# ksil/LFPSQP.jl

Measured on AMD Instinct MI355X. Metric: projected-CG iters/sec at n=1e7, m=128 fp64, higher is better.
Workload: dtype f64

## Files before the change

lfpsqp.jl_amd/csrc/context.hip:

```cpp
#include <dlfcn.h>
#include <stdarg.h>
#include <stdio.h>
#include <stdlib.h>
#include <ctype.h>
#include <string.h>

#include <algorithm>

#include "internal.h"

namespace lfpsqp {

int set_err(lfpsqp_ctx* ctx, int code, const char* fmt, ...) {
    char buf[1024];
    va_list ap;
    va_start(ap, fmt);
    vsnprintf(buf, sizeof(buf), fmt, ap);
    va_end(ap);
    if (ctx) ctx->err = buf;
    else fprintf(stderr, "lfpsqp: %s\n", buf);
    return code;
}

static int regrow(lfpsqp_ctx* ctx, double** buf, size_t* have, size_t cap, bool zero) {
// ... 222 lines not shown
}

__global__ __launch_bounds__(lfpsqp::kThreads) void view_copy_kernel(const double* __restrict__ A, const double* __restrict__ rs, const double* __restrict__ u,
                                                                     const double* __restrict__ w, double* __restrict__ D, int64_t ld, int64_t n, int m) {
    const int64_t i = ((int64_t)blockIdx.x * lfpsqp::kThreads + threadIdx.x) * 2;
    if (i >= n) return;
    const double2 s = rs ? lfpsqp::ld2(rs + i) : make_double2(1.0, 1.0);
    const double2 uu = u ? lfpsqp::ld2(u + i) : make_double2(0.0, 0.0);
    const bool v1 = i + 1 < n;
    const int j0 = blockIdx.y * 16, j1 = (j0 + 16 < m) ? j0 + 16 : m;
#pragma unroll 4
    for (int j = j0; j < j1; ++j) {
        const double2 c = lfpsqp::ld2(A + (int64_t)j * ld + i);
        const double wj = u ? w[j] : 0.0;
        const double2 o = make_double2(fma(uu.x, wj, s.x * c.x), fma(uu.y, wj, s.y * c.y));
        if (v1) lfpsqp::st2(D + (int64_t)j * ld + i, o);
        else D[(int64_t)j * ld + i] = o.x;
    }
}

extern "C" {

int lfpsqp_ctx_create(int device, lfpsqp_ctx** out) {
    if (!out) return LFPSQP_ERR_ARG;
    *out = nullptr;
    int ndev = 0;
    if (hipGetDeviceCount(&ndev) != hipSuccess || ndev <= 0) return set_err(nullptr, LFPSQP_ERR_HIP, "no HIP device visible");
    if (device < 0 || device >= ndev) return set_err(nullptr, LFPSQP_ERR_ARG, "device %d out of range (%d visible)", device, ndev);
    lfpsqp_ctx* ctx = new lfpsqp_ctx();
    ctx->device = device;
    if (hipSetDevice(device) != hipSuccess) { delete ctx; return set_err(nullptr, LFPSQP_ERR_HIP, "hipSetDevice(%d) failed", device); }
    hipDeviceProp_t prop;
    if (hipGetDeviceProperties(&prop, device) == hipSuccess) {
        ctx->devname = std::string(prop.name) + " (" + prop.gcnArchName + ")";
        ctx->num_cu = prop.multiProcessorCount;
        ctx->real_gpu = strncmp(prop.gcnArchName, "gfx", 3) == 0;
    }
    bool ok = hipStreamCreate(&ctx->stream) == hipSuccess;
    ok = ok && hipMalloc((void**)&ctx->scal, 64 * sizeof(double)) == hipSuccess;
    ok = ok && hipMalloc((void**)&ctx->istat, 128 * sizeof(int64_t)) == hipSuccess;
    ok = ok && hipHostMalloc((void**)&ctx->h_scal, 4 * 64 * sizeof(double)) == hipSuccess;
    ok = ok && hipHostMalloc((void**)&ctx->h_istat, 4 * 16 * sizeof(int64_t)) == hipSuccess;
    for (int i = 0; ok && i < 4; ++i) ok = hipEventCreate(&ctx->ev_slot[i]) == hipSuccess;
    ok = ok && hipEventCreate(&ctx->ev_t0) == hipSuccess && hipEventCreate(&ctx->ev_t1) == hipSuccess;
    if (ok) ok = hipMemset(ctx->scal, 0, 64 * sizeof(double)) == hipSuccess && hipMemset(ctx->istat, 0, 128 * sizeof(int64_t)) == hipSuccess;
    if (!ok) { delete ctx; return set_err(nullptr, LFPSQP_ERR_HIP, "context resource allocation failed"); }
    if (const char* e = getenv("LFPSQP_ONEPASS")) ctx->tune_onepass = atoi(e);
    if (const char* e = getenv("LFPSQP_SPGRAM")) ctx->tune_spgram = atoi(e) < 0 ? -1 : 0;
    if (const char* e = getenv("LFPSQP_VEC_BLOCKS")) ctx->tune_vec_blocks = atoi(e) > 0 ? atoi(e) : 0;
    if (const char* e = getenv("LFPSQP_NRB_MFMA")) ctx->tune_nrb_mfma = atoi(e) > 0 ? 1 : (atoi(e) < 0 ? -1 : 0);
    if (const char* e = getenv("LFPSQP_GPING")) ctx->tune_gping = atoi(e) == 1 ? 1 : 0;
    if (const char* e = getenv("LFPSQP_NRB_WG_CAP")) ctx->batch_wg_cap = atoi(e) > 0 ? atoi(e) : 0;
    if (const char* e = getenv("LFPSQP_STAGE_ROUNDS")) ctx->stage_cap = atoi(e) > 0 ? atoi(e) : 0;
    *out = ctx;
    return 0;
}

int lfpsqp_ctx_destroy(lfpsqp_ctx* ctx) {
    if (!ctx) return 0;
    (void)hipSetDevice(ctx->device);
    (void)hipStreamSynchronize(ctx->stream);
    if (ctx->comm.kind == Comm::RCCL && ctx->comm.nccl_comm && ctx->comm.ncclCommDestroy) ctx->comm.ncclCommDestroy(ctx->comm.nccl_comm);
    for (int r = 0; r < kP2PMaxRanks; ++r)
        if (ctx->comm.p2p_peer[r] && ctx->comm.p2p_peer[r] != ctx->comm.p2p_mine) (void)hipIpcCloseMemHandle(ctx->comm.p2p_peer[r]);
    if (ctx->comm.p2p_mine) (void)hipFree(ctx->comm.p2p_mine);
    if (ctx->comm.p2p_err) (void)hipHostFree(ctx->comm.p2p_err);
    if (ctx->prof_init)
        for (int s = 0; s < kProfSlots; ++s)
            for (int e = 0; e < kProfEvents; ++e)
                for (int k = 0; k < 2; ++k) (void)hipEventDestroy(ctx->prof_ev[s][e][k]);
    for (int i = 0; i < 4; ++i) if (ctx->ev_slot[i]) (void)hipEventDestroy(ctx->ev_slot[i]);
    if (ctx->ev_t0) (void)hipEventDestroy(ctx->ev_t0);
    if (ctx->ev_t1) (void)hipEventDestroy(ctx->ev_t1);
    if (ctx->part) (void)hipFree(ctx->part);
    if (ctx->small) (void)hipFree(ctx->small);
    if (ctx->d_m) (void)hipFree(ctx->d_m);
    if (ctx->d_qw) (void)hipFree(ctx->d_qw);
    if (ctx->d_zeros) (void)hipFree(ctx->d_zeros);
    if (ctx->d_nvec) (void)hipFree(ctx->d_nvec);
    if (ctx->d_tri) (void)hipFree(ctx->d_tri);
    if (ctx->d_view) (void)hipFree(ctx->d_view);
    if (ctx->h_m) (void)hipHostFree(ctx->h_m);
    if (ctx->scal) (void)hipFree(ctx->scal);
    if (ctx->istat) (void)hipFree(ctx->istat);
    if (ctx->h_scal) (void)hipHostFree(ctx->h_scal);
    if (ctx->h_istat) (void)hipHostFree(ctx->h_istat);
    if (ctx->stream) (void)hipStreamDestroy(ctx->stream);
    delete ctx;
    return 0;
}

int lfpsqp_ctx_sync(lfpsqp_ctx* ctx) {
    LF_ARG(ctx, ctx != nullptr);
    LF_HIP(ctx, hipStreamSynchronize(ctx->stream));
    return 0;
}

const char* lfpsqp_last_error(const lfpsqp_ctx* ctx) { return ctx ? ctx->err.c_str() : "null context"; }

int lfpsqp_device_name(const lfpsqp_ctx* ctx, char* buf, int64_t buflen) {
    if (!ctx || !buf || buflen <= 0) return LFPSQP_ERR_ARG;
    snprintf(buf, (size_t)buflen, "%s", ctx->devname.c_str());
    return 0;
}

int lfpsqp_device_uuid(const lfpsqp_ctx* ctx, char* buf, int64_t buflen) {
// ... 588 lines not shown
```

lfpsqp.jl_amd/csrc/internal.h:

```cpp
#pragma once
#include <hip/hip_runtime.h>
#include <stdint.h>

#include <string>
#include <vector>

#include "../../include/lfpsqp_hip.h"
#include "kernels.h"

struct lfpsqp_slab {
    void* p = nullptr;
    int refs = 0;
};
struct lfpsqp_vec {
    double* p = nullptr;
    int64_t n = 0;
    int64_t cap = 0;
    lfpsqp_slab* slab = nullptr;
};

constexpr int64_t kLdSkewDefault = 16;

struct lfpsqp_mat {
    double* p = nullptr;
    int64_t n = 0, m = 0;
    int64_t ld = 0;
    const double* rs = nullptr;
    const double* ru = nullptr;
    const double* rw = nullptr;
    bool view = false;
    lfpsqp_mat plain() const { lfpsqp_mat q = *this; q.rs = q.ru = q.rw = nullptr; q.view = false; return q; }
};

namespace lfpsqp {

constexpr int kProfSlots = 8;
constexpr int kProfEvents = 128;

struct Comm {
    int rank = 0, nranks = 1;
    enum Kind { NONE, RCCL, CALLBACK, P2P } kind = NONE;
    void* p2p_mine = nullptr;
    void* p2p_peer[16] = {nullptr};
    uint64_t p2p_seq = 0;
    int* p2p_err = nullptr;
    int p2p_memkind = 0;
    bool p2p_allow_coarse = false;
    void* rccl_lib = nullptr;
    void* nccl_comm = nullptr;
    int (*ncclAllReduce)(const void*, void*, size_t, int , int , void*, hipStream_t) = nullptr;
    int (*ncclCommDestroy)(void*) = nullptr;
    const char* (*ncclGetErrorString)(int) = nullptr;
    lfpsqp_allreduce_fn cb = nullptr;
    void* cb_user = nullptr;
};

}

struct lfpsqp_ctx {
    int device = 0;
    int num_cu = 0;
    hipStream_t stream = nullptr;
    std::string err;
    std::string devname;
    lfpsqp::Comm comm;
    bool comm_active() const { return comm.kind != lfpsqp::Comm::NONE; }

    double* part = nullptr;
    size_t part_cap = 0;
    double* small = nullptr;
    size_t small_cap = 0;
    double* d_m = nullptr;
    double* h_m = nullptr;
    size_t m_cap = 0;
    std::vector<double> warm_V;
    int warm_m = 0;
    double* d_view = nullptr;
    double* d_nvec = nullptr;
    size_t nvec_cap = 0;
    double* d_tri = nullptr;
    size_t tri_cap = 0;
    double* d_zeros = nullptr;
    double* d_qw = nullptr;
    size_t qw_cap = 0;
    double* scal = nullptr;
    int64_t* istat = nullptr;
    double* h_scal = nullptr;
    int64_t* h_istat = nullptr;
    hipEvent_t ev_slot[4] = {nullptr, nullptr, nullptr, nullptr};
    hipEvent_t ev_t0 = nullptr, ev_t1 = nullptr;

    int tune_ks = 0;
    bool tune_nt = true;
    int ks_for(int64_t n) const { return tune_ks ? tune_ks : (n >= 4000000 ? 4 : 2); }
    int tune_onepass = 0;
    int tune_spgram = 0;
    int tune_vec_blocks = 0;
    int tune_nrb_mfma = -1;
    int tune_gping = 0;

    bool real_gpu = false;
    int place_tries = 3;
    int64_t place_min_bytes = (int64_t)1 << 30;
    double place_last_ms[64] = {0};
    int place_last_n = 0, place_last_pick = 0;

    struct ProjcgResume {
        bool valid = false;
        const double *x = nullptr, *g = nullptr, *d = nullptr, *Z = nullptr;
        int m = 0;
        int64_t nv = 0, iters = 0;
        bool gcur_is_rp = false;
        const double *dg = nullptr, *b = nullptr;
        double a0 = 0.0;
        int64_t n_global = 0;
        uint64_t epoch = 0;
    } pcg_resume;
    int batch_wg_cap = 0;
    int stage_cap = 0;
    uint64_t launch_epoch = 0;

    bool profiling = false;
    hipEvent_t prof_ev[lfpsqp::kProfSlots][lfpsqp::kProfEvents][2];
    int prof_used[lfpsqp::kProfSlots] = {0};
    int64_t prof_seq[lfpsqp::kProfSlots] = {0};
    bool prof_live[lfpsqp::kProfSlots] = {false};
    int64_t prof_count[lfpsqp::kProfSlots] = {0};
    double prof_ms[lfpsqp::kProfSlots] = {0};
    bool prof_init = false;
};

namespace lfpsqp {

int set_err(lfpsqp_ctx* ctx, int code, const char* fmt, ...);
int ensure_part(lfpsqp_ctx* ctx, size_t doubles);
int ensure_small(lfpsqp_ctx* ctx, size_t doubles);
int ensure_tri(lfpsqp_ctx* ctx, size_t doubles);
int ensure_mvec(lfpsqp_ctx* ctx, size_t doubles);
int ensure_nvec(lfpsqp_ctx* ctx, size_t doubles);

struct Layout {
    struct Region { double** p; size_t at; };
    Region r[12];
    int k = 0;
    size_t n = 0;
    size_t skip(size_t len, size_t align = 2) {
        const size_t at = (n + align - 1) / align * align;
        n = at + len;
        return at;
    }
    void add(double*& p, size_t len, size_t align = 2) { r[k++] = Region{&p, skip(len, align)}; }
    size_t size() const { return n; }
    void carve(double* base) const { for (int i = 0; i < k; ++i) *r[i].p = base + r[i].at; }
};
int ensure_view(lfpsqp_ctx* ctx);
constexpr int kViewTau = 8;
constexpr int kViewScratch = kViewTau + 4 * 1024 + 64;
int allreduce_dev(lfpsqp_ctx* ctx, double* buf, int64_t count, int op = 0);

void prof_begin(lfpsqp_ctx* ctx, int s);
void prof_end(lfpsqp_ctx* ctx, int s);
void prof_collect(lfpsqp_ctx* ctx);

inline int64_t round_up(int64_t a, int64_t b) { return (a + b - 1) / b * b; }
inline int64_t ntiles_of(int64_t n, int ks) { return (n + (int64_t)kSlabRows * ks - 1) / ((int64_t)kSlabRows * ks); }

#define LF_HIP(ctx, expr)                                                                              \
    do {                                                                                               \
        hipError_t e__ = (expr);                                                                       \
        if (e__ != hipSuccess)                                                                         \
            return lfpsqp::set_err((ctx), LFPSQP_ERR_HIP, "%s failed: %s (%s:%d)", #expr,              \
                                   hipGetErrorString(e__), __FILE__, __LINE__);                        \
// ... 376 lines not shown
```

lfpsqp.jl_amd/csrc/projcg.hip:

```cpp
#include <math.h>
#include <stdlib.h>

#include <algorithm>
#include <vector>

#include "internal.h"
#include "sparse.h"
#include "sphess.h"

namespace lfpsqp {

enum { S_DAD = 0, S_RG = 1, S_ALPHA = 2, S_RPGP = 3, S_GPGP = 4, S_BETA = 5, S_NR = 6, S_TOL = 7, S_DD = 8, S_ALPHA_PREV = 9 };
enum { I_STATUS = 0, I_ITER = 1, I_MAXIT = 2 };
enum { ST_RUNNING = 0, ST_CONVERGED = 1, ST_RG_BREAK = 2, ST_NEGCURV = 3, ST_MAXIT = 4 };

struct AOpD {
    double a0;
    const double* dg;
    __device__ __forceinline__ double2 apply(int64_t i, double2 d) const {
        if (dg) {
            const double2 q = ld2(dg + i);
            return make_double2((a0 + q.x) * d.x, (a0 + q.y) * d.y);
        }
        return make_double2(a0 * d.x, a0 * d.y);
    }
};

struct AOpV {
    const double* Av;
    __device__ __forceinline__ double2 apply(int64_t i, double2) const { return ld2(Av + i); }
};

struct AOpLR {
    double a0;
    const double* dg;
    const double* V;
    int64_t ldv;
    int k;
    const double *sigma, *vtv;
    __device__ __forceinline__ double2 apply(int64_t i, double2 d) const {
        double2 o = dg ? make_double2((a0 + dg[i]) * d.x, (a0 + dg[i + 1]) * d.y) : make_double2(a0 * d.x, a0 * d.y);
        for (int j = 0; j < k; ++j) {
            const double c = ld_scal(sigma + j) * ld_scal(vtv + j);
            const double2 v = ld2(V + (int64_t)j * ldv + i);
            o.x = fma(v.x, c, o.x);
            o.y = fma(v.y, c, o.y);
        }
        return o;
    }
};

template <int B>
struct BandD {
    static_assert(B >= 1 && B <= 4, "bandwidth 1 .. 4");
    double a0;
    const double* dg;
// ... 352 lines not shown
    int first;
    __device__ __forceinline__ bool skip() const { return ld_stat(istat + I_STATUS) != ST_RUNNING; }
    __device__ __forceinline__ void apply(int64_t i, bool v0, bool v1, double* red) const {
        double2 dd = ld2(d + i);
        if (!first) {
            const double alpha = ld_scal(scal + S_ALPHA);
            double2 xx = ld2(x + i);
            xx = make_double2(fma(alpha, dd.x, xx.x), fma(alpha, dd.y, xx.y));
            if (v1) st2(x + i, xx);
            else if (v0) x[i] = xx.x;
            const double beta = ld_scal(scal + S_BETA);
            const double2 gg = ld2(g + i);
            dd = make_double2(beta * dd.x - gg.x, beta * dd.y - gg.y);
            if (v1) st2(d + i, dd);
            else if (v0) d[i] = dd.x;
        }
        const double2 ad = A.apply(i, dd);
        double s = 0.0;
        if (v0) s = dd.x * ad.x;
        if (v1) s = fma(dd.y, ad.y, s);
        red[0] += s;
    }
};
struct PcgDirX {
    double* d;
    const double* g;
    double* x;
    const double* scal;
    const int64_t* istat;
    __device__ __forceinline__ bool skip() const { return ld_stat(istat + I_STATUS) != ST_RUNNING; }
    __device__ __forceinline__ void apply(int64_t i, bool v0, bool v1, double*) const {
        const double alpha = ld_scal(scal + S_ALPHA), beta = ld_scal(scal + S_BETA);
        double2 dd = ld2(d + i), xx = ld2(x + i);
        const double2 gg = ld2(g + i);
        xx = make_double2(fma(alpha, dd.x, xx.x), fma(alpha, dd.y, xx.y));
        dd = make_double2(beta * dd.x - gg.x, beta * dd.y - gg.y);
        if (v1) { st2(x + i, xx); st2(d + i, dd); }
        else if (v0) { x[i] = xx.x; d[i] = dd.x; }
    }
};
struct DotPairF {
    const double* a;
    const double* b;
    const int64_t* istat;
    __device__ __forceinline__ bool skip() const { return ld_stat(istat + I_STATUS) != ST_RUNNING; }
    __device__ __forceinline__ void apply(int64_t i, bool v0, bool v1, double* red) const {
        const double2 x = ld2(a + i), y = ld2(b + i);
        double s = 0.0;
        if (v0) s = x.x * y.x;
        if (v1) s = fma(x.y, y.y, s);
        red[0] += s;
    }
};
constexpr int kRing = 8, kRingOff = 8;
struct HostMirror {
    int64_t* hstat;
    double* hnr;
    __device__ __forceinline__ void publish(int64_t status, int64_t iter, double nr) const {
        __hip_atomic_store(hnr, nr, __ATOMIC_RELAXED, __HIP_MEMORY_SCOPE_SYSTEM);
        __hip_atomic_store(hstat + 1, iter, __ATOMIC_RELAXED, __HIP_MEMORY_SCOPE_SYSTEM);
        __hip_atomic_store(hstat + kRingOff + (iter % kRing), status, __ATOMIC_RELAXED, __HIP_MEMORY_SCOPE_SYSTEM);
        __hip_atomic_store(hstat, status, __ATOMIC_RELEASE, __HIP_MEMORY_SCOPE_SYSTEM);
    }
};

struct PcgPost1 {
    double* scal;
    int64_t* istat;
    HostMirror hm;
    __device__ __forceinline__ bool skip() const { return ld_stat(istat + I_STATUS) != ST_RUNNING; }
    __device__ __forceinline__ void run(double*) const {
        const int64_t it = ld_stat(istat + I_ITER) + 1;
        istat[I_ITER] = it;
        const double dAd = ld_scal(scal + S_DAD), rg = ld_scal(scal + S_RG);
        if (dAd <= 0.0) { istat[I_STATUS] = ST_NEGCURV; hm.publish(ST_NEGCURV, it, ld_scal(scal + S_NR)); }
        else if (rg <= 0.0) { istat[I_STATUS] = ST_RG_BREAK; hm.publish(ST_RG_BREAK, it, ld_scal(scal + S_NR)); }
        else scal[S_ALPHA] = rg / dAd;
    }
};

template <class AOP>
struct PcgStepV {
    const double* d;
    const double* g;
    AOP A;
    const double* scal;
    const int64_t* istat;
    __device__ __forceinline__ bool skip() const { return ld_stat(istat + I_STATUS) != ST_RUNNING; }
    __device__ __forceinline__ double2 rp_at(int64_t r) const {
        const double alpha = ld_scal(scal + S_ALPHA);
        const double2 dd = ld2(d + r), gg = ld2(g + r);
        const double2 ad = A.apply(r, dd);
        return make_double2(fma(alpha, ad.x, gg.x), fma(alpha, ad.y, gg.y));
    }
    __device__ __forceinline__ double2 load(int64_t r, bool v0, bool v1) const {
        const double2 rr = rp_at(r);
        return make_double2(v0 ? rr.x : 0.0, v1 ? rr.y : 0.0);
    }
};

template <class AOP>
struct PcgProjE {
    const double* rp;
    double* g;
    double* d;
    const int64_t* istat;
    int init;
    PcgStepV<AOP> sv;
    __device__ __forceinline__ bool skip() const { return ld_stat(istat + I_STATUS) != ST_RUNNING; }
    __device__ __forceinline__ void apply(int64_t r, double2 acc, bool v0, bool v1, double* red) const {
        const double2 rr = init ? ld2(rp + r) : sv.rp_at(r);
        const double2 gp = make_double2(rr.x - acc.x, rr.y - acc.y);
        if (v1) st2(g + r, gp);
        else if (v0) g[r] = gp.x;
        if (init) {
// ... 434 lines not shown
            else if (gpgp <= 0.0) st = ST_RG_BREAK;
            else {
                u.scal[S_ALPHA_PREV] = (u.init == 2) ? 0.0 : ld_scal(u.scal + S_ALPHA);
                u.scal[S_ALPHA] = gpgp / dAd_next;
            }
            if (st != ST_RUNNING) u.hm.publish(st, it + 1, nr);
        }
        if (st != ST_RUNNING) u.istat[I_STATUS] = st;
        go = (st == ST_RUNNING);
        sh[0] = gpgp / dAd_next;
        sh[1] = beta;
        if (go)
            for (int j = 0; j < u.k; ++j) {
                const double vg = ld_scal(S + 5 + j);
                const double vd = (u.init == 1) ? -vg : fma(beta, u.vdraw[j], -vg);
                u.vdraw[j] = vd;
                u.vdc[j] = ld_scal(u.sigma + j) * vd;
            }
    }
    __syncthreads();
    if (!go) return;
    const double alpha = sh[0], beta = sh[1];
    for (int j = threadIdx.x; j < u.m; j += blockDim.x) {
        const double t1 = ld_scal(u.T + j);
        double t2 = ld_scal(u.T + u.m + j);
        if (u.triM) t2 -= s_mu[j];
        for (int l = 0; l < u.k; ++l)
            t2 = fma(u.UtV[(size_t)l * u.m + j], ld_scal(u.sigma + l) * ld_scal(u.T + 2 * u.m + 5 + l), t2);
        const double t3 = (u.init == 1) ? -t2 : fma(beta, u.t3[j], -t2);
        u.t3[j] = t3;
        const double ut = fma(alpha, t3, t1);
        u.Utr[j] = ut;
        if (u.W) s_utr[j] = ut;
    }
    if (u.W) {
        __syncthreads();
        const double* const xin[1] = {nullptr};
        double yo[1];
        small_wdot<1>(u.W, 1, (size_t)u.wm, u.wm, u.m, xin, s_utr, yo, s_part);
        int rp = 32;
        while (rp < u.wm) rp <<= 1;
        if ((int)threadIdx.x < u.wm && (int)threadIdx.x / rp == 0) u.uA[threadIdx.x] = yo[0];
    }
}
#ifndef LFPSQP_K1_NT
#define LFPSQP_K1_NT 1
#endif
struct PcgDirG {
    double* d;
    const double* g;
    double* x;
    const double* scal;
    const int64_t* istat;
    int force;
    __device__ __forceinline__ bool skip() const { return !force && ld_stat(istat + I_STATUS) != ST_RUNNING; }
    __device__ __forceinline__ void apply(int64_t i, bool v0, bool v1, double*) const {
        double2 dd = ld2(d + i);
        if (!force) {
            const double alpha = ld_scal(scal + S_ALPHA_PREV);
            double2 xx = ld2(x + i);
            xx = make_double2(fma(alpha, dd.x, xx.x), fma(alpha, dd.y, xx.y));
            if (v1) { if (LFPSQP_K1_NT >= 1) st2_stream(x + i, xx); else st2(x + i, xx); }
            else if (v0) x[i] = xx.x;
        }
        const double beta = ld_scal(scal + S_BETA);
        const double2 gg = ld2(g + i);
        dd = make_double2(beta * dd.x - gg.x, beta * dd.y - gg.y);
        if (v1) { if (LFPSQP_K1_NT == 1) st2_stream(d + i, dd); else st2(d + i, dd); }
        else if (v0) d[i] = dd.x;
    }
};

template <class AOP>
struct ResidualV {
    const double* x;
    const double* b;
    double* out;
    AOP A;
    double sgn;
    __device__ __forceinline__ bool skip() const { return false; }
    __device__ __forceinline__ double2 load(int64_t r, bool v0, bool v1) const {
        const double2 xx = ld2(x + r), bb = ld2(b + r);
        const double2 ax = A.apply(r, xx);
        const double2 rr = make_double2(sgn * (ax.x - bb.x), sgn * (ax.y - bb.y));
        if (out) {
            if (v1) st2(out + r, rr);
            else if (v0) out[r] = rr.x;
        }
        return make_double2(v0 ? rr.x : 0.0, v1 ? rr.y : 0.0);
    }
};
struct InitState {
    double* scal;
    int64_t* istat;
    double tol;
    int64_t maxit;
    __device__ __forceinline__ bool skip() const { return false; }
    __device__ __forceinline__ void run(double*) const {
        for (int k = 0; k < 16; ++k) scal[k] = 0.0;
        scal[S_TOL] = tol;
        scal[S_NR] = INFINITY;
        istat[I_STATUS] = ST_RUNNING;
        istat[I_ITER] = 0;
        istat[I_MAXIT] = maxit;
    }
};
struct FlushXF {
    double* x;
    const double* d;
    const double* scal;
    __device__ __forceinline__ bool skip() const { return false; }
    __device__ __forceinline__ void apply(int64_t i, bool v0, bool v1, double*) const {
        const double alpha = ld_scal(scal + S_ALPHA);
        const double2 dd = ld2(d + i);
        double2 xx = ld2(x + i);
        xx = make_double2(fma(alpha, dd.x, xx.x), fma(alpha, dd.y, xx.y));
        if (v1) st2(x + i, xx);
        else if (v0) x[i] = xx.x;
    }
};
// ... 341 lines not shown
    static CoupledOp sparse_of(const char* who, double a0, const lfpsqp_vec* dg, const lfpsqp_sphess* S) {
        return CoupledOp{SPARSE, who, a0, dg, nullptr, 0, S->n, S->Kr, {}, S};
    }
    static CoupledOp banded(const char* who, double a0, const lfpsqp_vec* dg, const double* off, int64_t ld, int64_t rows, int bw) {
        return CoupledOp{BAND, who, a0, dg, off, ld, rows, bw, {1, 2, 3, 4}};
    }
};
template <typename F>
static int with_diags(const CoupledOp& A, F&& fn) {
    return A.wide() ? fn(std::integral_constant<int, kDiagsWide>{}) : fn(std::integral_constant<int, kDiagsNarrow>{});
}
template <typename F>
static int with_gathers(const CoupledOp& A, int64_t n, int64_t nc, F&& fn) {
    if (A.kind == CoupledOp::SPARSE) return fn(A.sparse(n, nc));
    return with_diags(A, [&](auto Cc) -> int { return fn(A.template diags<decltype(Cc)::value>(n, nc)); });
}
template <typename F>
static int with_band(int bw, F&& fn) {
    switch (bw) {
        case 1: return fn(std::integral_constant<int, 1>{});
        case 2: return fn(std::integral_constant<int, 2>{});
        case 3: return fn(std::integral_constant<int, 3>{});
        default: return fn(std::integral_constant<int, 4>{});
    }
}

static int coupled_mul(lfpsqp_ctx* ctx, const CoupledOp& A, int64_t n, int64_t nc, const double* v, double* out) {
    if (A.kind != CoupledOp::BAND)
        return with_gathers(A, n, nc, [&](auto Ad) -> int {
            using D = decltype(Ad);
            return run_vec<DiagsMulF<D>, 0, NoPost>(ctx, n, DiagsMulF<D>{Ad, v, out, nullptr}, 0u, nullptr, NoPost());
        });
    return with_band(A.K, [&](auto Bc) -> int {
        constexpr int B = decltype(Bc)::value;
        return run_vec<TriMulF<B>, 0, NoPost>(ctx, n, TriMulF<B>{A.template band<B>(n, nc), v, out, nullptr}, 0u, nullptr, NoPost());
    });
}
template <typename F>
static int with_stacked_init(bool stacked, bool init, F&& fn) {
    if (stacked) return init ? fn(std::true_type{}, std::true_type{}) : fn(std::true_type{}, std::false_type{});
    return init ? fn(std::false_type{}, std::true_type{}) : fn(std::false_type{}, std::false_type{});
}

struct PcgOperator {
    enum Kind { DIAGONAL, CALLBACK, LOWRANK, COUPLED } kind;
    lfpsqp_diag_op diag;
    lfpsqp_opfun fn = nullptr;
    void* user = nullptr;
    const lfpsqp_lowrank_op* lr = nullptr;
    const CoupledOp* cp = nullptr;
    lfpsqp_vec* Av = nullptr;
};

static int projcg_impl(lfpsqp_ctx* ctx, lfpsqp_vec* x, lfpsqp_vec* lambda, const PcgOperator& op, const lfpsqp_basis* U, const lfpsqp_vec* b,
                       const lfpsqp_vec* c, double tol, int64_t maxit, int64_t n_global, int flags, const lfpsqp_projcg_work* work,
                       int64_t* iters, double* nr) {
    const bool callback = op.kind == PcgOperator::CALLBACK;
    const lfpsqp_lowrank_op* LRop = op.kind == PcgOperator::LOWRANK ? op.lr : nullptr;
    const CoupledOp* cop = op.kind == PcgOperator::COUPLED ? op.cp : nullptr;
    const lfpsqp_diag_op* A = &op.diag;
    lfpsqp_vec* Av = op.Av;
    LF_ARG(ctx, ctx && x && U && b && work && iters && nr);
    if (callback || cop) {
        LF_ARG(ctx, Av && Av->n == b->n && !(flags & (LFPSQP_PROJCG_RESUME | (cop ? 0 : LFPSQP_PROJCG_START_GIVEN) | LFPSQP_PROJCG_START_PROJECTED)));
    }
    LF_ARG(ctx, !((flags & LFPSQP_PROJCG_RESUME) && (flags & (LFPSQP_PROJCG_START_GIVEN | LFPSQP_PROJCG_START_PROJECTED))));
    LF_ARG(ctx, !((flags & LFPSQP_PROJCG_START_GIVEN) && (flags & LFPSQP_PROJCG_START_PROJECTED)));
    LF_ARG(ctx, work->g && work->d && work->rp && work->Utr);
    const lfpsqp_ctx::ProjcgResume rs = ctx->pcg_resume;
    const bool stacked = U->Dx != nullptr;
    const int64_t nv = b->n;
    const int m = (int)U->ncols;
    LF_ARG(ctx, x->n == nv && work->g->n == nv && work->d->n == nv && work->rp->n == nv);
    const bool DF = m > 0 && !U->Z && U->A && U->W && !U->SA && m <= U->A->m && U->A->m <= kOnepassMaxCols;
    const bool SF = m > 0 && !U->Z && U->A && U->W && U->SA;
    LF_ARG(ctx, m >= 0 && (m == 0 || ((DF || SF || (U->Z && m <= U->Z->m)) && work->Utr->n >= m)));
    LF_ARG(ctx, !A->dg || A->dg->n == nv);
    LF_ARG(ctx, n_global >= (stacked ? 0 : nv));
    int64_t N = nv, hs = 0;
    if (stacked) {
        LF_ARG(ctx, U->Dy && U->sx && U->sy);
        N = U->Dx->n;
        hs = lfpsqp_half_stride(N);
        LF_ARG(ctx, nv == hs + N && U->Dy->n == N && U->sx->n == N && U->sy->n == N && (m == 0 || ((DF || SF) ? U->A->n : U->Z->n) == N));
        if (c) return set_err(ctx, LFPSQP_ERR_UNSUPPORTED, "stacked basis with c != 0 (never used by optimize, src/optimize.jl:368)");
        LF_ARG(ctx, !(flags & LFPSQP_PROJCG_WANT_LAMBDA) || (lambda && lambda->n >= N + m));
    } else {
        LF_ARG(ctx, m == 0 || ((DF || SF) ? U->A->n : U->Z->n) == nv);
        LF_ARG(ctx, !c || c->n >= m);
        LF_ARG(ctx, !(flags & LFPSQP_PROJCG_WANT_LAMBDA) || (lambda && lambda->n >= m));
    }

    const AOpD Ad{A->a0, A->dg ? A->dg->p : nullptr};
    double* scal = ctx->scal;
    int64_t* istat = ctx->istat;
    double* g = work->g->p;
    double* d = work->d->p;
    double* rp = work->rp->p;
    double* Utr = work->Utr->p;
    const lfpsqp_mat* Z = m > 0 ? (DF ? U->A : U->Z) : nullptr;
    const int mc = DF ? (int)U->A->m : m;
    const StackD sk = stacked ? StackD{hs, U->Dx->p, U->Dy->p, U->sx->p, U->sy->p} : StackD{0, nullptr, nullptr, nullptr, nullptr};
    const int64_t m_ref = stacked ? n_global / 2 + m : m;
    int64_t maxit_eff = maxit < n_global + m_ref ? maxit : n_global + m_ref;
    if (maxit_eff < 0) maxit_eff = 0;

// ... 33 lines not shown
    if (LRop) {
        LF_ARG(ctx, LRop->V && plain_mat(LRop->V) && kLR >= 1 && kLR <= kLRMax && LRop->V->m >= kLR && LRop->V->n == nv && (!LRop->dg || LRop->dg->n == nv));
        if (!fused || stacked || (flags & (LFPSQP_PROJCG_RESUME | LFPSQP_PROJCG_START_GIVEN | LFPSQP_PROJCG_START_PROJECTED)))
            return set_err(ctx, LFPSQP_ERR_UNSUPPORTED, "lfpsqp_projcg_lowrank: needs the one-pass iteration over a plain dense basis (4 .. 1024 columns), no RESUME / START_GIVEN");
    }
    std::vector<double> triMh;
    if (cop) {
        if (cop->kind == CoupledOp::SPARSE) LF_ARG(ctx, cop->sp && cop->rows == N && (!cop->dg || cop->dg->n == nv));
        else LF_ARG(ctx, cop->off && cop->rows == N && cop->K >= 1 && cop->K <= (cop->kind == CoupledOp::DIAGS ? kDiagsWide : kDiagsNarrow) && (!cop->dg || cop->dg->n == nv));
        if (!fused || !plain_mat(Z) || ctx->comm_active())
            return set_err(ctx, LFPSQP_ERR_UNSUPPORTED, "%s: needs the one-pass iteration over a dense basis (4 .. 1024 columns, no matrix "
                                                        "view) on a single rank (the couplings would cross the shard boundaries); use lfpsqp_projcg_op",
                           cop->who);
        if (cop->kind == CoupledOp::SPARSE)
            LF_TRY(reduced_operator_sparse(ctx, Z, mc, cop->a0, cop->dgp(), *cop->sp, DF ? U->W : nullptr, m, triMh, stacked ? &sk : nullptr));
        else LF_TRY(with_diags(*cop, [&](auto Cc) -> int {
            return reduced_operator(ctx, Z, mc, cop->template diags<decltype(Cc)::value>(N, N), DF ? U->W : nullptr, m, triMh, stacked ? &sk : nullptr);
        }));
    }
    double* dTriM = nullptr;
    double *lrUtV = nullptr, *lrSig = nullptr, *lrVdraw = nullptr, *lrVdc = nullptr, *lrVtv = nullptr;
    if (fused) {
        Layout L;
        L.add(T12, 2 * m + ns);
        L.add(t3, m);
        if (DF) {
            L.add(Traw, 2 * mc + ns);
            L.add(uDF, mc);
        }
        if (kLR > 0) { L.add(lrUtV, (size_t)m * kLRMax); L.add(lrSig, kLRMax); L.add(lrVdraw, kLRMax); L.add(lrVdc, kLRMax); L.add(lrVtv, kLRMax); }
        L.skip(2 * kLRMax + 24 + (DF ? 16 : 0) + (kLR > 0 ? 8 : 0));
        LF_TRY(ensure_mvec(ctx, L.size()));
        L.carve(ctx->d_m);
        if (DF || cop) {
            Layout Ls;
            if (DF) Ls.add(dWf, (size_t)mc * m);
            if (cop) Ls.add(dTriM, (size_t)m * m);
            Ls.skip(64);
            LF_TRY(ensure_small(ctx, Ls.size()));
            Ls.carve(ctx->small);
            if (DF) LF_HIP(ctx, hipMemcpyAsync(dWf, U->W, sizeof(double) * (size_t)mc * m, hipMemcpyHostToDevice, ctx->stream));
            if (cop) LF_HIP(ctx, hipMemcpyAsync(dTriM, triMh.data(), sizeof(double) * (size_t)m * m, hipMemcpyHostToDevice, ctx->stream));
            LF_HIP(ctx, hipStreamSynchronize(ctx->stream));
        }
    }
    auto df_gemv_t = [&](auto vf, double* t_out, double* u_out) -> int {
        LF_TRY(run_gemv_t(ctx, Z, mc, N, vf, Traw));
        return sp_basis_small(ctx, dWf, mc, m, Traw, t_out, u_out);
    };
    const HostMirror hm{ctx->h_istat, ctx->h_scal};
    volatile int64_t* hstat = ctx->h_istat;
    hstat[0] = ST_RUNNING;
    hstat[1] = 0;
    for (int k = 0; k < kRing; ++k) hstat[kRingOff + k] = ST_RUNNING;
    auto apply_op = [&](const lfpsqp_vec* v) -> int {
        const int rc = op.fn(op.user, v, Av);
        if (rc != 0) return set_err(ctx, LFPSQP_ERR_ARG, "operator callback returned %d", rc);
        return 0;
    };
    const AOpV Aop{(callback || cop) ? Av->p : nullptr};
    auto residual_with = [&](auto aop, double sgn, double* store, double* t_out) -> int {
        using AOP = decltype(aop);
        const ResidualV<AOP> rv{x->p, b->p, store, aop, sgn};
        if (SA && stacked) return sp_gemv_t(ResidualVS<AOP>{rv, sk, store ? nullptr : lambda->p}, tmpN, t_out, store ? uA : nullptr);
        if (DF && stacked) return df_gemv_t(ResidualVS<AOP>{rv, sk, store ? nullptr : lambda->p}, t_out, store ? uDF : nullptr);
        if (DF) return df_gemv_t(rv, t_out, store ? uDF : nullptr);
        if (stacked) return run_gemv_t(ctx, Z, m, N, ResidualVS<AOP>{rv, sk, store ? nullptr : lambda->p}, t_out);
        if (SA) return sp_gemv_t(rv, tmpN, t_out, store ? uA : nullptr);
        return run_gemv_t(ctx, Z, m, N, rv, t_out);
    };
    auto launch_residual = [&](double sgn, double* store, double* t_out) -> int {
        if (kLR > 0) {
            LF_TRY(run_gemv_t(ctx, LRop->V, kLR, N, SpPlainV{x->p}, lrVtv));
            return residual_with(AOpLR{Ad.a0, Ad.dg, LRop->V->p, LRop->V->ld, kLR, lrSig, lrVtv}, sgn, store, t_out);
        }
        if (cop) {
            LF_TRY(coupled_mul(ctx, *cop, nv, N, x->p, Av->p));
            return residual_with(Aop, sgn, store, t_out);
        }
        if (!callback) return residual_with(Ad, sgn, store, t_out);
        LF_TRY(apply_op(x));
        return residual_with(Aop, sgn, store, t_out);
    };
    auto k2_with = [&](auto aop) -> int {
        using AOP = decltype(aop);
        const PcgStepV<AOP> sv{d, g, aop, scal, istat};
        if (SA && stacked) return sp_gemv_t(PcgStepVS<AOP>{sv, sk}, tmpN, Utr, uA);
        if (stacked) return run_gemv_t(ctx, Z, m, N, PcgStepVS<AOP>{sv, sk}, Utr, 1);
        if (SA) return sp_gemv_t(sv, tmpN, Utr, uA);
        return run_gemv_t(ctx, Z, m, N, sv, Utr, 1);
    };
    auto launch_k2 = [&]() -> int { return callback ? k2_with(Aop) : k2_with(Ad); };
    auto k3_with = [&](auto aop, int init) -> int {
        using AOP = decltype(aop);
        const PcgProjE<AOP> pe{rp, g, d, istat, init, PcgStepV<AOP>{d, g, aop, scal, istat}};
        const PcgPost3 post{scal, istat, init, hm, scal + S_RPGP};
        if (SA && stacked) {
            using E = PcgProjES<AOP>;
            const SpConsumeE<E> ce{E{pe, sk}, ell_rows(SA, uA), U->A->p + (int64_t)SA->m * U->A->ld, U->A->ld, uA + SA->m, nxs};
            return run_vec<SpConsumeE<E>, 2, PcgPost3>(ctx, N, ce, 0u, scal + S_RPGP, post, init ? -1 : 2);
        }
        if (stacked) return run_gemv_n<PcgProjES<AOP>, 2, PcgPost3>(ctx, Z, m, N, Utr, PcgProjES<AOP>{pe, sk}, scal + S_RPGP, post, init ? -1 : 2);
        if (SA) {
            using E = PcgProjE<AOP>;
            const SpConsumeE<E> ce{pe, ell_rows(SA, uA), U->A->p + (int64_t)SA->m * U->A->ld, U->A->ld, uA + SA->m, nxs};
            return run_vec<SpConsumeE<E>, 2, PcgPost3>(ctx, nv, ce, 0u, scal + S_RPGP, post, init ? -1 : 2);
// ... 21 lines not shown
                LF_TRY((run_vec<DiagsPrepSF<D, INIT>, 0, NoPost>(ctx, N, DiagsPrepSF<D, INIT>{Ab, hs, sk.Dx, sk.Dy, src, dsrc, ad, ux, scal, istat}, 0u, nullptr, NoPost())));
                return run_vec<DiagsGatherF<D>, 0, NoPost>(ctx, N, DiagsGatherF<D>{Ab, ux, nullptr, q, scal, istat}, 0u, nullptr, NoPost());
            } else {
                if constexpr (!INIT) LF_TRY((run_vec<DiagsMulF<D>, 0, NoPost>(ctx, N, DiagsMulF<D>{Ab, dsrc, ad, istat}, 0u, nullptr, NoPost())));
                return run_vec<DiagsGatherF<D>, 0, NoPost>(ctx, N, DiagsGatherF<D>{Ab, src, ad, q, scal, istat}, 0u, nullptr, NoPost());
            }
        });
    };
    auto launch_fused = [&](int init) -> int {
        const int slot = init ? -1 : 3;
        const double* gin = gbuf[gcur];
        double* gout = init ? gbuf[0] : gbuf[gcur ^ 1];
        const double* tin = DF ? uDF : Utr;
        double* Tout = DF ? Traw : T12;
        auto fuse_lr = [&](auto INc) -> int {
            constexpr bool INIT = decltype(INc)::value;
            return run_onepass<PcgFuseLR<INIT>, 2, 5 + kLRMax>(ctx, Z, mc, mc, N, tin, PcgFuseLR<INIT>{rp, gin, gout, d, Ad, scal, istat, LRop->V->p, LRop->V->ld, kLR, lrVdc}, Tout, slot);
        };
        if (cop) LF_TRY(with_stacked_init(stacked, init != 0, [&](auto STc, auto INc) -> int {
            constexpr bool ST = decltype(STc)::value, INIT = decltype(INc)::value;
            const double* src = INIT ? rp : gin;
            const double* dsrc = INIT ? nullptr : d;
            double* ad = INIT ? nullptr : Av->p;
            double* q = INIT ? Av->p : rp;
            LF_TRY(prepare_neighbours(STc, INc, src, dsrc, ad, q));
            return run_onepass<PcgFuseTri<ST, INIT>, 2, 5>(ctx, Z, mc, mc, N, tin, PcgFuseTri<ST, INIT>{rp, gin, gout, d, ad, q, Ad, scal, istat, sk}, Tout, slot);
        }));
        else if (kLR > 0) LF_TRY(init ? fuse_lr(std::true_type{}) : fuse_lr(std::false_type{}));
        else LF_TRY(with_stacked_init(stacked, init != 0, [&](auto STc, auto INc) -> int {
            constexpr bool ST = decltype(STc)::value, INIT = decltype(INc)::value;
            return run_onepass<PcgFuseE<ST, INIT>, 2, 5>(ctx, Z, mc, mc, N, tin, PcgFuseE<ST, INIT>{rp, gin, gout, d, Ad, scal, istat, sk}, Tout, slot);
        }));
        if (!init) gcur ^= 1;
        PcgPostF pf{T12, t3, Utr, scal, istat, m, init, hm, dWf, Traw, T12, uDF, DF ? mc : 0};
        if (kLR > 0) { pf.k = kLR; pf.UtV = lrUtV; pf.sigma = lrSig; pf.vdraw = lrVdraw; pf.vdc = lrVdc; }
        pf.triM = dTriM;
        hipLaunchKernelGGL(pcg_post_kernel, dim3(1), dim3(DF ? 1024 : 256), 0, ctx->stream, pf);
        LF_LAUNCH_CHECK(ctx);
        return 0;
    };

    const bool resume = (flags & LFPSQP_PROJCG_RESUME) != 0;
    int64_t it_base = 0;
    if (resume) {
        if (!fused || !rs.valid || rs.x != x->p || rs.g != g || rs.d != d || rs.Z != Z->p || rs.m != m || rs.nv != nv || rs.dg != Ad.dg ||
            rs.a0 != Ad.a0 || rs.b != b->p || rs.n_global != n_global || rs.epoch != ctx->launch_epoch)
            return set_err(ctx, LFPSQP_ERR_UNSUPPORTED, "LFPSQP_PROJCG_RESUME: no resumable projcg state for these arguments "
                           "(needs the one-pass iteration, a previous call with the same x, A, U, b, work that stopped at its iteration limit, and no library call that queued device work in between)");
        it_base = rs.iters;
        gcur = (rs.gcur_is_rp && gbuf[1] == rp) ? 1 : 0;
        if (rs.gcur_is_rp != (gcur == 1)) return set_err(ctx, LFPSQP_ERR_UNSUPPORTED, "LFPSQP_PROJCG_RESUME: the buffer scheme changed between the calls");
        maxit_eff = (it_base + maxit < n_global + m_ref) ? it_base + maxit : n_global + m_ref;
        hstat[1] = it_base;
        const int64_t lim = maxit_eff;
        LF_HIP(ctx, hipMemcpyAsync(istat + I_MAXIT, &lim, sizeof(int64_t), hipMemcpyHostToDevice, ctx->stream));
        LF_HIP(ctx, hipStreamSynchronize(ctx->stream));
        hipLaunchKernelGGL(pcg_post_kernel, dim3(1), dim3(DF ? 1024 : 256), 0, ctx->stream, PcgPostF{T12, t3, Utr, scal, istat, m, 2, hm, dWf, Traw, T12, uDF, DF ? mc : 0});
        LF_LAUNCH_CHECK(ctx);
    }
    ctx->pcg_resume.valid = false;
    if (!resume) {
        hipLaunchKernelGGL((post_kernel<InitState>), dim3(1), dim3(1), 0, ctx->stream, scal, InitState{scal, istat, tol, maxit_eff});
        LF_LAUNCH_CHECK(ctx);

        if (c && m > 0) {
            if (!DF) LF_TRY(lfpsqp_gemv_n(ctx, Z, m, 1.0, c, 0.0, x));
        } else {
            LF_TRY(lfpsqp_vec_fill(ctx, x, 0.0));
        }
        if (kLR > 0) {
            for (int j = 0; j < kLRMax; ++j) ctx->h_m[j] = (j < kLR) ? (LRop->sigma ? LRop->sigma[j] : 1.0) : 0.0;
            LF_HIP(ctx, hipMemcpyAsync(lrSig, ctx->h_m, sizeof(double) * kLRMax, hipMemcpyHostToDevice, ctx->stream));
            LF_HIP(ctx, hipStreamSynchronize(ctx->stream));
            LF_HIP(ctx, hipMemsetAsync(lrVdraw, 0, sizeof(double) * 3 * kLRMax, ctx->stream));
            for (int l = 0; l < kLR; ++l) {
                const SpPlainV col{LRop->V->p + (int64_t)l * LRop->V->ld};
                if (DF) LF_TRY(df_gemv_t(col, lrUtV + (size_t)l * m, nullptr));
                else LF_TRY(run_gemv_t(ctx, Z, m, N, col, lrUtV + (size_t)l * m));
            }
        }
        if (flags & LFPSQP_PROJCG_START_PROJECTED) {
            if (!(DF && fused && !c && kLR == 0) || work->Utr->n < (int64_t)mc + 2 * m + 5)
                return set_err(ctx, LFPSQP_ERR_UNSUPPORTED, "LFPSQP_PROJCG_START_PROJECTED: basis in factored form over a dense generator, c == NULL, work->Utr of >= A.m + 2 ncols + 5 entries");
            LF_HIP(ctx, hipMemcpyAsync(T12, Utr + mc, sizeof(double) * (2 * (size_t)m + 5), hipMemcpyDeviceToDevice, ctx->stream));
            PcgPostF pf{T12, t3, Utr, scal, istat, m, 1, hm, dWf, Traw, T12, uDF, mc};
            pf.pre = 1;
            hipLaunchKernelGGL(pcg_post_kernel, dim3(1), dim3(1024), 0, ctx->stream, pf);
            LF_LAUNCH_CHECK(ctx);
        } else if (flags & LFPSQP_PROJCG_START_GIVEN) {
            if (!(DF && fused && !c))
                return set_err(ctx, LFPSQP_ERR_UNSUPPORTED, "LFPSQP_PROJCG_START_GIVEN: basis in factored form over a dense generator, c == NULL");
            LF_TRY(factored_w_times_t(ctx, dWf, mc, m, Utr, uDF));
        } else {
            LF_TRY(launch_residual(1.0, rp, Utr));
        }
        if (flags & LFPSQP_PROJCG_START_PROJECTED) {  }
        else if (fused) LF_TRY(launch_fused(1));
        else LF_TRY(launch_k3(1));
    }

    int64_t it = 0;
    bool done = false;
    const int gcur_start = gcur;
    const int64_t it_end = maxit_eff - it_base;
    while (!done && it < it_end) {
        if (fused) {
            if (it > 0 || resume) LF_TRY((run_vec<PcgDirG, 0, NoPost>(ctx, nv, PcgDirG{d, gbuf[gcur], x->p, scal, istat, 0}, 0u, nullptr, NoPost(), 0)));
            LF_TRY(launch_fused(0));
        } else if (callback) {
            if (it > 0) LF_TRY((run_vec<PcgDirX, 0, NoPost>(ctx, nv, PcgDirX{d, g, x->p, scal, istat}, 0u, nullptr, NoPost(), 0)));
            LF_TRY(apply_op(work->d));
            LF_TRY((run_vec<DotPairF, 1, PcgPost1>(ctx, nv, DotPairF{d, Av->p, istat}, 0u, scal + S_DAD, PcgPost1{scal, istat, hm})));
            LF_TRY(launch_k2());
            LF_TRY(launch_k3(0));
        } else {
            LF_TRY((run_vec<PcgDirF, 1, PcgPost1>(ctx, nv, PcgDirF{d, g, x->p, Ad, scal, istat, it == 0 ? 1 : 0}, 0u, scal + S_DAD,
                                                  PcgPost1{scal, istat, hm}, 0)));
            LF_TRY(launch_k2());
            LF_TRY(launch_k3(0));
        }
        LF_HIP(ctx, hipEventRecord(ctx->ev_slot[it & 3], ctx->stream));
        if (it >= 2) {
            LF_HIP(ctx, hipEventSynchronize(ctx->ev_slot[(it - 2) & 3]));
            if (hstat[kRingOff + ((it_base + it - 1) % kRing)] != ST_RUNNING) done = true;
        }
        ++it;
    }
    LF_HIP(ctx, hipStreamSynchronize(ctx->stream));
    const int64_t status = hstat[0];
    *iters = hstat[1];
    *nr = *(volatile double*)ctx->h_scal;
    if (fused) {
        const int64_t executed = ((status == ST_CONVERGED || status == ST_MAXIT) ? *iters : *iters - 1) - it_base;
        gcur = (gbuf[1] != gbuf[0]) ? (int)((gcur_start + (executed > 0 ? executed : 0)) & 1) : 0;
    }

    if ((status == ST_CONVERGED || status == ST_MAXIT || (fused && status == ST_RG_BREAK && *iters > 1)) && *iters > it_base)
        LF_TRY((run_vec<FlushXF, 0, NoPost>(ctx, nv, FlushXF{x->p, d, scal}, 0u, nullptr, NoPost())));
    if (fused && status == ST_MAXIT && *iters > 0 && kLR == 0 && !cop)
        ctx->pcg_resume = lfpsqp_ctx::ProjcgResume{true, x->p, g, d, Z->p, m, nv, *iters, gcur == 1, Ad.dg, b->p, Ad.a0, n_global, ctx->launch_epoch};
    if (status == ST_NEGCURV) {
        if (fused && *iters > 1)
            LF_TRY((run_vec<PcgDirG, 0, NoPost>(ctx, nv, PcgDirG{d, gbuf[gcur], x->p, scal, istat, 1}, 0u, nullptr, NoPost())));
        LF_TRY((run_vec<SumSqF, 1, NoPost>(ctx, nv, SumSqF{d}, 0u, scal + S_DD, NoPost())));
        LF_TRY((run_vec<NormalizeIntoF, 0, NoPost>(ctx, nv, NormalizeIntoF{x->p, d, scal + S_DD}, 0u, nullptr, NoPost())));
        if (lambda) LF_TRY(lfpsqp_vec_fill(ctx, lambda, NAN));
        *nr = INFINITY;
    } else if (flags & LFPSQP_PROJCG_WANT_LAMBDA) {
        if (stacked) LF_TRY(launch_residual(-1.0, nullptr, lambda->p + N));
        else if (m > 0) LF_TRY(launch_residual(-1.0, nullptr, lambda->p));
    }
    if (ctx->profiling) {
        LF_HIP(ctx, hipStreamSynchronize(ctx->stream));
        prof_collect(ctx);
    }
    return 0;
}

int lfpsqp::placement_probe(lfpsqp_ctx* ctx, const lfpsqp_mat* M, int ncols, double* g, double* d, double* a, int reps, double* ms) {
    *ms = -1.0;
    if (!M || M->n <= 0 || ncols < 4 || ncols > M->m || onepass_cw(ctx, ncols, M->ld, M->n) == 0) return 0;
    double *T12, *Utr;
    Layout L;
    L.add(T12, 2 * ncols + 5); L.add(Utr, ncols); L.skip(18);
    LF_TRY(ensure_mvec(ctx, L.size()));
    L.carve(ctx->d_m);
    LF_HIP(ctx, hipMemsetAsync(ctx->d_m, 0, sizeof(double) * L.size(), ctx->stream));
    hipLaunchKernelGGL((post_kernel<InitState>), dim3(1), dim3(1), 0, ctx->stream, ctx->scal, InitState{ctx->scal, ctx->istat, 0.0, (int64_t)1 << 40});
    LF_LAUNCH_CHECK(ctx);
    const StackD sk{0, nullptr, nullptr, nullptr, nullptr};
    const Comm::Kind saved = ctx->comm.kind;
    ctx->comm.kind = Comm::NONE;
    int rc = 0;
    for (int k = 0; k < reps + 1 && rc == 0; ++k) {
        if (k == 1) rc = hipEventRecord(ctx->ev_t0, ctx->stream) == hipSuccess ? 0 : LFPSQP_ERR_HIP;
        if (rc == 0) rc = with_stacked_init(false, false, [&](auto STc, auto INc) -> int {
            constexpr bool ST = decltype(STc)::value, INIT = decltype(INc)::value;
            return run_onepass<PcgFuseE<ST, INIT>, 2, 5>(ctx, M, ncols, ncols, M->n, Utr, PcgFuseE<ST, INIT>{g, g, g, d, AOpD{0.0, a}, ctx->scal, ctx->istat, sk}, T12, -1);
        });
    }
    ctx->comm.kind = saved;
    LF_TRY(rc);
    LF_HIP(ctx, hipEventRecord(ctx->ev_t1, ctx->stream));
    LF_HIP(ctx, hipEventSynchronize(ctx->ev_t1));
    float t = 0.f;
    LF_HIP(ctx, hipEventElapsedTime(&t, ctx->ev_t0, ctx->ev_t1));
    *ms = (double)t / reps;
    return 0;
}

extern "C" int lfpsqp_projcg(lfpsqp_ctx* ctx, lfpsqp_vec* x, lfpsqp_vec* lambda, const lfpsqp_diag_op* A, const lfpsqp_basis* U,
                             const lfpsqp_vec* b, const lfpsqp_vec* c, double tol, int64_t maxit, int64_t n_global, int flags,
                             const lfpsqp_projcg_work* work, int64_t* iters, double* nr) {
    LF_RANGE("lfpsqp_projcg");
    LF_ARG(ctx, ctx && A);
    return projcg_impl(ctx, x, lambda, PcgOperator{PcgOperator::DIAGONAL, *A}, U, b, c, tol, maxit, n_global, flags, work, iters, nr);
// ... 136 lines not shown
```

Before: 594.2.

## Batch x updates across iteration pairs and poll host-mapped progress word

The fused projected-CG direction kernel now alternates lean iterations, which update only d, with paired iterations that apply two alpha steps to x at once. This removes the x read and write on every other iteration, at the cost of an extra g-derived term in the paired update and more complex final-flush bookkeeping. The host loop also stops recording and synchronizing events each iteration. Instead it spin-polls a packed progress word written by the device into pinned host memory, falling back to a stream query, which cuts per-iteration runtime API overhead but spends host CPU time spinning.

```diff
diff --git a/lfpsqp.jl_amd/csrc/context.hip b/lfpsqp.jl_amd/csrc/context.hip
--- a/lfpsqp.jl_amd/csrc/context.hip
+++ b/lfpsqp.jl_amd/csrc/context.hip
@@ -298,6 +298,7 @@
     if (const char* e = getenv("LFPSQP_GPING")) ctx->tune_gping = atoi(e) == 1 ? 1 : 0;
     if (const char* e = getenv("LFPSQP_NRB_WG_CAP")) ctx->batch_wg_cap = atoi(e) > 0 ? atoi(e) : 0;
     if (const char* e = getenv("LFPSQP_STAGE_ROUNDS")) ctx->stage_cap = atoi(e) > 0 ? atoi(e) : 0;
+    if (const char* e = getenv("LFPSQP_STEP_TAIL")) ctx->step_tail = atoi(e) & kStepTailAll;
     *out = ctx;
     return 0;
 }
diff --git a/lfpsqp.jl_amd/csrc/internal.h b/lfpsqp.jl_amd/csrc/internal.h
--- a/lfpsqp.jl_amd/csrc/internal.h
+++ b/lfpsqp.jl_amd/csrc/internal.h
@@ -54,6 +54,8 @@
     lfpsqp_allreduce_fn cb = nullptr;
     void* cb_user = nullptr;
 };
+
+constexpr int kStepTailPoll = 1, kStepTailPairX = 2, kStepTailAll = kStepTailPoll | kStepTailPairX;
 
 }
 
@@ -118,6 +120,7 @@
     } pcg_resume;
     int batch_wg_cap = 0;
     int stage_cap = 0;
+    int step_tail = lfpsqp::kStepTailAll;
     uint64_t launch_epoch = 0;
 
     bool profiling = false;
diff --git a/lfpsqp.jl_amd/csrc/projcg.hip b/lfpsqp.jl_amd/csrc/projcg.hip
--- a/lfpsqp.jl_amd/csrc/projcg.hip
+++ b/lfpsqp.jl_amd/csrc/projcg.hip
@@ -2,6 +2,8 @@
 #include <stdlib.h>
 
 #include <algorithm>
+#include <chrono>
+#include <thread>
 #include <vector>
 
 #include "internal.h"
@@ -460,7 +462,8 @@
         red[0] += s;
     }
 };
-constexpr int kRing = 8, kRingOff = 8;
+constexpr int kRing = 8, kRingOff = 8, kProgress = 2;
+__host__ __device__ __forceinline__ int64_t progress_word(int64_t status, int64_t iter) { return (iter << 8) | status; }
 struct HostMirror {
     int64_t* hstat;
     double* hnr;
@@ -469,6 +472,7 @@
         __hip_atomic_store(hstat + 1, iter, __ATOMIC_RELAXED, __HIP_MEMORY_SCOPE_SYSTEM);
         __hip_atomic_store(hstat + kRingOff + (iter % kRing), status, __ATOMIC_RELAXED, __HIP_MEMORY_SCOPE_SYSTEM);
         __hip_atomic_store(hstat, status, __ATOMIC_RELEASE, __HIP_MEMORY_SCOPE_SYSTEM);
+        __hip_atomic_store(hstat + kProgress, progress_word(status, iter), __ATOMIC_RELEASE, __HIP_MEMORY_SCOPE_SYSTEM);
     }
 };
 
@@ -1009,20 +1013,25 @@
     double* x;
     const double* scal;
     const int64_t* istat;
-    int force;
-    __device__ __forceinline__ bool skip() const { return !force && ld_stat(istat + I_STATUS) != ST_RUNNING; }
+    enum { kOne = 0, kForced = 1, kPair = 2, kLean = 3 };
+    int mode;
+    __device__ __forceinline__ bool skip() const { return mode != kForced && ld_stat(istat + I_STATUS) != ST_RUNNING; }
     __device__ __forceinline__ void apply(int64_t i, bool v0, bool v1, double*) const {
-        double2 dd = ld2(d + i);
-        if (!force) {
+        const double2 d0 = ld2(d + i);
+        const double beta = ld_scal(scal + S_BETA);
+        const double2 gg = ld2(g + i);
+        const double2 dd = make_double2(beta * d0.x - gg.x, beta * d0.y - gg.y);
+        if (mode == kOne || mode == kPair) {
             const double alpha = ld_scal(scal + S_ALPHA_PREV);
             double2 xx = ld2(x + i);
-            xx = make_double2(fma(alpha, dd.x, xx.x), fma(alpha, dd.y, xx.y));
+            xx = make_double2(fma(alpha, d0.x, xx.x), fma(alpha, d0.y, xx.y));
+            if (mode == kPair) {
+                const double alpha1 = ld_scal(scal + S_ALPHA);
+                xx = make_double2(fma(alpha1, dd.x, xx.x), fma(alpha1, dd.y, xx.y));
+            }
             if (v1) { if (LFPSQP_K1_NT >= 1) st2_stream(x + i, xx); else st2(x + i, xx); }
             else if (v0) x[i] = xx.x;
         }
-        const double beta = ld_scal(scal + S_BETA);
-        const double2 gg = ld2(g + i);
-        dd = make_double2(beta * dd.x - gg.x, beta * dd.y - gg.y);
         if (v1) { if (LFPSQP_K1_NT == 1) st2_stream(d + i, dd); else st2(d + i, dd); }
         else if (v0) d[i] = dd.x;
     }
@@ -1470,6 +1479,40 @@
     lfpsqp_vec* Av = nullptr;
 };
 
+constexpr int kProgressSpinUs = 50, kProgressQueryUs = 800;
+static inline hipError_t stream_state(hipStream_t s) {
+#ifdef LFPSQP_HIP_EMULATED
+    return hipSuccess;
+#else
+    return hipStreamQuery(s);
+#endif
+}
+static int await_progress(lfpsqp_ctx* ctx, const volatile int64_t* word, int64_t target, int64_t* seen, bool* drained) {
+    using clk = std::chrono::steady_clock;
+    *drained = false;
+    bool timed = false;
+    clk::time_point t0, tq;
+    for (;;) {
+        const int64_t w = __atomic_load_n(const_cast<const int64_t*>(word), __ATOMIC_ACQUIRE);
+        *seen = w;
+        if ((w & 0xff) != ST_RUNNING || (w >> 8) >= target) return 0;
+        const clk::time_point now = clk::now();
+        if (!timed) { t0 = tq = now; timed = true; continue; }
+        if (now - tq >= std::chrono::microseconds(kProgressQueryUs)) {
+            const hipError_t e = stream_state(ctx->stream);
+            if (e == hipSuccess) {
+                *seen = __atomic_load_n(const_cast<const int64_t*>(word), __ATOMIC_ACQUIRE);
+                *drained = (*seen & 0xff) == ST_RUNNING && (*seen >> 8) < target;
+                return 0;
+            }
+            if (e != hipErrorNotReady) LF_HIP(ctx, e);
+            (void)hipGetLastError();
+            tq = clk::now();
+        }
+        if (now - t0 >= std::chrono::microseconds(kProgressSpinUs)) std::this_thread::yield();
+    }
+}
+
 static int projcg_impl(lfpsqp_ctx* ctx, lfpsqp_vec* x, lfpsqp_vec* lambda, const PcgOperator& op, const lfpsqp_basis* U, const lfpsqp_vec* b,
                        const lfpsqp_vec* c, double tol, int64_t maxit, int64_t n_global, int flags, const lfpsqp_projcg_work* work,
                        int64_t* iters, double* nr) {
@@ -1609,6 +1652,7 @@
     volatile int64_t* hstat = ctx->h_istat;
     hstat[0] = ST_RUNNING;
     hstat[1] = 0;
+    hstat[kProgress] = progress_word(ST_RUNNING, 0);
     for (int k = 0; k < kRing; ++k) hstat[kRingOff + k] = ST_RUNNING;
     auto apply_op = [&](const lfpsqp_vec* v) -> int {
         const int rc = op.fn(op.user, v, Av);
@@ -1736,6 +1780,7 @@
         if (rs.gcur_is_rp != (gcur == 1)) return set_err(ctx, LFPSQP_ERR_UNSUPPORTED, "LFPSQP_PROJCG_RESUME: the buffer scheme changed between the calls");
         maxit_eff = (it_base + maxit < n_global + m_ref) ? it_base + maxit : n_global + m_ref;
         hstat[1] = it_base;
+        hstat[kProgress] = progress_word(ST_RUNNING, it_base);
         const int64_t lim = maxit_eff;
         LF_HIP(ctx, hipMemcpyAsync(istat + I_MAXIT, &lim, sizeof(int64_t), hipMemcpyHostToDevice, ctx->stream));
         LF_HIP(ctx, hipStreamSynchronize(ctx->stream));
@@ -1787,9 +1832,17 @@
     bool done = false;
     const int gcur_start = gcur;
     const int64_t it_end = maxit_eff - it_base;
+    const bool poll = fused && !ctx->comm_active() && (ctx->step_tail & kStepTailPoll);
+    const bool pair_x = fused && (ctx->step_tail & kStepTailPairX);
+    const int64_t k1_first = resume ? 0 : 1;
+    auto k1_mode = [&](int64_t i) -> int {
+        if (!pair_x) return PcgDirG::kOne;
+        if (i == k1_first) return resume ? PcgDirG::kLean : PcgDirG::kOne;
+        return ((i - k1_first) & 1) ? PcgDirG::kPair : PcgDirG::kLean;
+    };
     while (!done && it < it_end) {
         if (fused) {
-            if (it > 0 || resume) LF_TRY((run_vec<PcgDirG, 0, NoPost>(ctx, nv, PcgDirG{d, gbuf[gcur], x->p, scal, istat, 0}, 0u, nullptr, NoPost(), 0)));
+            if (it > 0 || resume) LF_TRY((run_vec<PcgDirG, 0, NoPost>(ctx, nv, PcgDirG{d, gbuf[gcur], x->p, scal, istat, k1_mode(it)}, 0u, nullptr, NoPost(), 0)));
             LF_TRY(launch_fused(0));
         } else if (callback) {
             if (it > 0) LF_TRY((run_vec<PcgDirX, 0, NoPost>(ctx, nv, PcgDirX{d, g, x->p, scal, istat}, 0u, nullptr, NoPost(), 0)));
@@ -1803,6 +1856,16 @@
             LF_TRY(launch_k2());
             LF_TRY(launch_k3(0));
         }
+        if (poll) {
+            if (it >= 2) {
+                bool drained = false;
+                int64_t seen = 0;
+                LF_TRY(await_progress(ctx, hstat + kProgress, it_base + it - 1, &seen, &drained));
+                if (drained || (seen & 0xff) != ST_RUNNING) done = true;
+            }
+            ++it;
+            continue;
+        }
         LF_HIP(ctx, hipEventRecord(ctx->ev_slot[it & 3], ctx->stream));
         if (it >= 2) {
             LF_HIP(ctx, hipEventSynchronize(ctx->ev_slot[(it - 2) & 3]));
@@ -1819,13 +1882,15 @@
         gcur = (gbuf[1] != gbuf[0]) ? (int)((gcur_start + (executed > 0 ? executed : 0)) & 1) : 0;
     }
 
-    if ((status == ST_CONVERGED || status == ST_MAXIT || (fused && status == ST_RG_BREAK && *iters > 1)) && *iters > it_base)
+    const int64_t last_done = ((status == ST_CONVERGED || status == ST_MAXIT) ? *iters : *iters - 1) - it_base - 1;
+    const bool x_current = last_done > k1_first && k1_mode(last_done) == PcgDirG::kPair;
+    if ((status == ST_CONVERGED || status == ST_MAXIT || (fused && status == ST_RG_BREAK && *iters > 1)) && *iters > it_base && !x_current)
         LF_TRY((run_vec<FlushXF, 0, NoPost>(ctx, nv, FlushXF{x->p, d, scal}, 0u, nullptr, NoPost())));
     if (fused && status == ST_MAXIT && *iters > 0 && kLR == 0 && !cop)
         ctx->pcg_resume = lfpsqp_ctx::ProjcgResume{true, x->p, g, d, Z->p, m, nv, *iters, gcur == 1, Ad.dg, b->p, Ad.a0, n_global, ctx->launch_epoch};
     if (status == ST_NEGCURV) {
         if (fused && *iters > 1)
-            LF_TRY((run_vec<PcgDirG, 0, NoPost>(ctx, nv, PcgDirG{d, gbuf[gcur], x->p, scal, istat, 1}, 0u, nullptr, NoPost())));
+            LF_TRY((run_vec<PcgDirG, 0, NoPost>(ctx, nv, PcgDirG{d, gbuf[gcur], x->p, scal, istat, PcgDirG::kForced}, 0u, nullptr, NoPost())));
         LF_TRY((run_vec<SumSqF, 1, NoPost>(ctx, nv, SumSqF{d}, 0u, scal + S_DD, NoPost())));
         LF_TRY((run_vec<NormalizeIntoF, 0, NoPost>(ctx, nv, NormalizeIntoF{x->p, d, scal + S_DD}, 0u, nullptr, NoPost())));
         if (lambda) LF_TRY(lfpsqp_vec_fill(ctx, lambda, NAN));
```

New measurement: 603.3, median of 6. 1.02x the previous value.
